# YuxinxinChen/dlrm-yx

Measured on AMD Instinct MI355X. Metric: DLRM samples/sec fwd+bwd at 1/2/4/8 MI355X; embedding HBM GB/s vs peak, higher is better.
Workload: dtype fp32; 1 GPU; mlperf_terabyte_synthetic; global_batch=2048, local_batch=2048, tables=26, rows_total=54063992, emb_dim=128, lookups_per_bag=1, optimizer=sgd, parallelism=table-sharded emb x1 + dp1, hip_graph=True, capture=whole, bot_sched=auto, tbe_role=True, bottom_parts=0, head_role=True, early_sort=True, feature_pad=False

## Files before the change

### dlrm-yx_amd/csrc/gemm.hip

```cpp
#include <cstdlib>
#include <cstring>
#include <type_traits>

#include "common.hpp"
#include "tbe_bwd_roles.hpp"

#ifndef DLRM_GEMM_STAMP
#define DLRM_GEMM_STAMP(slot)
#endif

namespace {

using f32x16 = __attribute__((ext_vector_type(16))) float;
using f32x4 = __attribute__((ext_vector_type(4))) float;
constexpr int kThreads = 256;
constexpr int kMaxSplit = 32;
constexpr int kMaxGroup = 6;
constexpr int64_t kTicketCap = 16384;
constexpr int kBK = 32;
constexpr int kRasterRows = 4;

struct GemmParams {
  int64_t M, N, K;
  float alpha;
// ... 6 lines not shown
  int epi;
  const float* bias;
  const float* aux;
  int64_t ldaux;
  int64_t ones_col;
  int layout;
  int tiles_m, tiles_n;
  int splits;
  int block0;
  int64_t kchunk;
  float* ws;
  int* counters;
  int mode;
  float* part;
  const float* alpha_dev;
};

struct GemmGroup {
  GemmParams p[kMaxGroup];
  int n;
  int total;
};

__device__ __forceinline__ int swz_kc(int r) {
  return ((r >> 1) & 7) ^ (((unsigned)((r & 15) - 4) < 8u) ? 2 : 0);
}

template <int MN, int BKT, bool KC, bool VEC, int NT, bool SWZ = false>
struct Stage {
  static_assert(!SWZ || (BKT % 32 == 0 && MN >= 32), "swizzled images: BKT 32 U, MN >= 32");
// ... 154 lines not shown
  asm("v_add_f32 %0, %1, %2" : "=v"(r) : "v"(a), "v"(b));
  return r;
}

__device__ __forceinline__ int xcd_remap(int bid, int nwg) {
  const int xcd = bid % 8;
  const int q = nwg / 8, r = nwg % 8;
  return (xcd < r ? xcd * (q + 1) : r * (q + 1) + (xcd - r) * q) + bid / 8;
}

__device__ __forceinline__ float apply_epilogue(const GemmParams& p, int64_t row, int64_t col,
                                                float v) {
  float* cp = p.C + row * p.ldc + col;
  switch (p.epi) {
    case DLRM_EPI_BIAS:
      v += p.bias[col];
      break;
    case DLRM_EPI_BIAS_RELU:
      v = fmaxf(v + p.bias[col], 0.f);
      break;
    case DLRM_EPI_RELU:
      v = fmaxf(v, 0.f);
      break;
    case DLRM_EPI_DRELU:
      v = p.aux[row * p.ldaux + col] > 0.f ? v : 0.f;
      break;
    case DLRM_EPI_SGD:
      v = *cp - v;
      break;
    case DLRM_EPI_ACCUM:
      v = *cp + v;
      break;
    default:
      break;
// ... 9 lines not shown
  else if constexpr (EPI == DLRM_EPI_RELU) return fmaxf(v, 0.f);
  else if constexpr (EPI == DLRM_EPI_DRELU) return aux > 0.f ? v : 0.f;
  else if constexpr (EPI == DLRM_EPI_SGD) return old - v;
  else if constexpr (EPI == DLRM_EPI_ACCUM) return old + v;
  else return v;
}

__device__ __forceinline__ float buf_ld(__amdgpu_buffer_rsrc_t r, int off) {
  return __builtin_bit_cast(float, __builtin_amdgcn_raw_buffer_load_b32(r, off, 0, 0));
}
__device__ __forceinline__ void buf_st(float v, __amdgpu_buffer_rsrc_t r, int off) {
  __builtin_amdgcn_raw_buffer_store_b32(__builtin_bit_cast(unsigned int, v), r, off, 0, 0);
}
constexpr int kOob = 0x7ffffff0;

template <int EPI, int NE>
__device__ __forceinline__ void store_elems(const GemmParams& p, const int (&row)[NE],
                                            const int (&col)[NE], const bool (&ok)[NE],
                                            const float (&v)[NE]) {
  const __amdgpu_buffer_rsrc_t rc = __builtin_amdgcn_make_buffer_rsrc(
      (void*)p.C, (short)0, (int)(((p.M - 1) * p.ldc + p.ldc) * 4), 0x00020000);
  int off[NE];
#pragma unroll
  for (int q = 0; q < NE; ++q)
    off[q] = ok[q] && row[q] < p.M ? (int)(((int64_t)row[q] * p.ldc + col[q]) * 4) : kOob;
  float old[NE], aux[NE], bias[NE];
#pragma unroll
  for (int q = 0; q < NE; ++q) old[q] = aux[q] = bias[q] = 0.f;
  if constexpr (EPI == DLRM_EPI_SGD || EPI == DLRM_EPI_ACCUM) {
#pragma unroll
    for (int q = 0; q < NE; ++q) old[q] = buf_ld(rc, off[q]);
  }
  if constexpr (EPI == DLRM_EPI_DRELU) {
    const __amdgpu_buffer_rsrc_t ra = __builtin_amdgcn_make_buffer_rsrc(
        (void*)p.aux, (short)0, (int)(((p.M - 1) * p.ldaux + p.ldaux) * 4), 0x00020000);
#pragma unroll
    for (int q = 0; q < NE; ++q)
      aux[q] = buf_ld(ra, ok[q] && row[q] < p.M ? (int)(((int64_t)row[q] * p.ldaux + col[q]) * 4)
                                                : kOob);
  }
  if constexpr (EPI == DLRM_EPI_BIAS || EPI == DLRM_EPI_BIAS_RELU) {
#pragma unroll
    for (int q = 0; q < NE; ++q) bias[q] = ok[q] ? p.bias[col[q]] : 0.f;
  }
#pragma unroll
  for (int q = 0; q < NE; ++q) buf_st(epi_value<EPI>(v[q], old[q], aux[q], bias[q]), rc, off[q]);
}

__device__ __forceinline__ bool epi_fits(const GemmParams& p) {
  const int64_t lim = 0x7ff00000LL;
  return (p.M + 256) * p.ldc * 4 < lim &&
         (p.epi != DLRM_EPI_DRELU || (p.M + 256) * p.ldaux * 4 < lim);
}

template <int NE>
__device__ __forceinline__ void store_elems_any(const GemmParams& p, const int (&row)[NE],
                                                const int (&col)[NE], const bool (&ok)[NE],
                                                const float (&v)[NE]) {
  switch (p.epi) {
    case DLRM_EPI_BIAS: return store_elems<DLRM_EPI_BIAS>(p, row, col, ok, v);
    case DLRM_EPI_BIAS_RELU: return store_elems<DLRM_EPI_BIAS_RELU>(p, row, col, ok, v);
    case DLRM_EPI_RELU: return store_elems<DLRM_EPI_RELU>(p, row, col, ok, v);
    case DLRM_EPI_DRELU: return store_elems<DLRM_EPI_DRELU>(p, row, col, ok, v);
    case DLRM_EPI_SGD: return store_elems<DLRM_EPI_SGD>(p, row, col, ok, v);
    case DLRM_EPI_ACCUM: return store_elems<DLRM_EPI_ACCUM>(p, row, col, ok, v);
    default: return store_elems<DLRM_EPI_STORE>(p, row, col, ok, v);
  }
}


template <int BM, int BN, int NV, int FM>
__device__ __forceinline__ bool splitk_reduce(const GemmParams& p, int tile, int split,
                                              float (&v)[NV], float (&rs)[FM], int rs_row0,
                                              int rs_stride, bool rs_owner, float* smem) {
  if (p.splits <= 1) return true;
  constexpr int REC = BM * BN + BM;
  static_assert(NV % 4 == 0, "record chunks are float4");
  using u32x4 = __attribute__((ext_vector_type(4))) unsigned int;
  const int tid = threadIdx.x;
  float* tile_base = p.ws + (int64_t)tile * p.splits * REC;
  const __amdgpu_buffer_rsrc_t rr = __builtin_amdgcn_make_buffer_rsrc(
      (void*)tile_base, (short)0, (int)(p.splits * REC * 4), 0x00020000);
// ... 52 lines not shown
    load_rec(s + 1, t1, r1);
    add_rec(t0, r0, s == 0);
    add_rec(t1, r1, false);
  }
  if (s < p.splits) {
    float4 t0[NV / 4];
    float r0[FM];
    load_rec(s, t0, r0);
    add_rec(t0, r0, s == 0);
  }
  return true;
}

template <int BM, int BN, int WGM, int WGN, bool RS, int FM, int FN>
__device__ __forceinline__ void finish_tile(const GemmParams& p, float alpha,
                                            const f32x4 (&acc)[FM][FN], float (&rs)[FM], int tile,
                                            int split, int tn, int64_t m0, int64_t n0,
                                            float* smem) {
  constexpr int WM = BM / WGM, WN = BN / WGN;
  const int tid = threadIdx.x;
  const int wave = tid >> 6;
  const int lane = tid & 63;
  const int kq = lane >> 4;
  const int l16 = lane & 15;
  const int wm0 = (wave / WGN) * WM;
  const int wn0 = (wave % WGN) * WN;
  const bool rs_owner = RS && tn == 0 && (wave % WGN) == 0 && kq == 0;

  constexpr int NV = FM * FN * 4;
  float v[NV];
#pragma unroll
  for (int i = 0; i < FM; ++i)
#pragma unroll
// ... 42 lines not shown
      float* rslab = p.part + (int64_t)p.splits * p.M * p.N + (int64_t)split * p.M;
#pragma unroll
      for (int i = 0; i < FM; ++i) {
        const int64_t row = m0 + wm0 + i * 16 + l16;
        if (row < p.M) rslab[row] = rs[i];
      }
    }
    return;
  }
  if (!splitk_reduce<BM, BN, NV, FM>(p, tile, split, v, rs, wm0 + l16, 16, rs_owner, smem))
    return;
  if (epi_fits(p)) {
    int row[NV], col[NV];
    bool ok[NV];
    float w[NV];
#pragma unroll
    for (int i = 0; i < FM; ++i)
#pragma unroll
      for (int j = 0; j < FN; ++j)
#pragma unroll
        for (int r = 0; r < 4; ++r) {
          const int q = (i * FN + j) * 4 + r;
          row[q] = (int)(m0 + wm0 + i * 16 + 4 * kq + r);
          col[q] = (int)(n0 + wn0 + j * 16 + l16);
          ok[q] = col[q] < p.N;
          w[q] = __fmul_rn(alpha, v[q]);
        }
    store_elems_any<NV>(p, row, col, ok, w);
    if constexpr (RS) {
      int rrow[FM], rcol[FM];
      bool rok[FM];
      float rw[FM];
#pragma unroll
      for (int i = 0; i < FM; ++i) {
        rrow[i] = (int)(m0 + wm0 + i * 16 + l16);
        rcol[i] = (int)p.ones_col;
        rok[i] = rs_owner;
        rw[i] = __fmul_rn(alpha, rs[i]);
      }
      store_elems_any<FM>(p, rrow, rcol, rok, rw);
    }
    return;
  }
#pragma unroll
  for (int i = 0; i < FM; ++i)
#pragma unroll
    for (int j = 0; j < FN; ++j) {
      const int64_t col = n0 + wn0 + j * 16 + l16;
#pragma unroll
      for (int r = 0; r < 4; ++r) {
        const int64_t row = m0 + wm0 + i * 16 + 4 * kq + r;
        if (row < p.M && col < p.N) apply_epilogue(p, row, col, alpha * v[(i * FN + j) * 4 + r]);
      }
    }
  if (rs_owner) {
// ... 158 lines not shown
    if (!last) {
      mfma_step(ca, cb, KL - 1);
      const int g = u * KL + KL - 1;
      if (g < NS) {
        put_one(g, nbuf);
        fetch_any(g, kt + 2, fast);
      }
      __builtin_amdgcn_sched_barrier(0);
    } else {
      __syncthreads();
      read_frags(nbuf, 0, na, nb);
      __builtin_amdgcn_sched_barrier(0);
      mfma_step(ca, cb, KL - 1);
    }
  };
  float a1[FM][KL], b1[FN][KL];
  if constexpr (U == 1) {
    const std::true_type fast{};
    const std::false_type slow{};
    for (int kt = 0; kt < nk; kt += 2) {
      if (kb32 + (kt + 3) * BKT <= kend32)
        subtile(kt, 0, a, b, a1, b1, fast);
      else
        subtile(kt, 0, a, b, a1, b1, slow);
      DLRM_GEMM_STAMP(2 + kt);
      if (kt + 1 >= nk) break;
      if (kb32 + (kt + 4) * BKT <= kend32)
        subtile(kt + 1, 0, a1, b1, a, b, fast);
      else
        subtile(kt + 1, 0, a1, b1, a, b, slow);
      DLRM_GEMM_STAMP(3 + kt);
    }
  } else {
    for (int kt = 0; kt < nk; ++kt) {
#pragma unroll
      for (int u = 0; u < U; u += 2) {
        subtile(kt, u, a, b, a1, b1, std::false_type{});
        subtile(kt, u + 1, a1, b1, a, b, std::false_type{});
      }
    }
  }

#pragma unroll
  for (int i = 0; i < FM; ++i) {
    rs[i] += __shfl_xor(rs[i], 16, 64);
    rs[i] += __shfl_xor(rs[i], 32, 64);
  }
  DLRM_GEMM_STAMP(-2);
  finish_tile<BM, BN, WGM, WGN, RS>(p, alpha, acc, rs, tile, split, tn, m0, n0, smem);
  DLRM_GEMM_STAMP(-1);
}

__device__ __forceinline__ void reduce_body(const GemmParams& p, int lb) {
  const float alpha = dlrm_resolve_lr(p.alpha_dev, p.alpha);
  const int64_t MN = p.M * p.N;
  const int64_t i = (int64_t)lb * blockDim.x + threadIdx.x;
  const int64_t n4 = MN / 4;
  const int S = p.splits;
  if (i < n4) {
    const float4* src = reinterpret_cast<const float4*>(p.part) + i;
    const int64_t stride = MN / 4;
    float4 acc = src[0];
    for (int s0 = 1; s0 < S; s0 += 8) {
      float4 t[8];
// ... 184 lines not shown
  int64_t M, N, K;
  float alpha;
  const float *A, *B;
  int64_t lda, ldb;
  float* C;
  int64_t ldc;
  int32_t epi;
  const float* bias;
  const float* aux;
  int64_t ldaux;
  int64_t ones_col;
  int32_t mode = DLRM_GEMM_FULL;
  int32_t splits = 0;
  float* part = nullptr;
  const float* alpha_dev = nullptr;
};

inline bool aligned16(const void* p) { return (reinterpret_cast<uintptr_t>(p) & 15) == 0; }

bool pipe_ok(const Desc& d) {
  const bool a_kc = !d.trans_a, b_kc = d.trans_b != 0;
  const int64_t a_ext = a_kc ? (d.M - 1) * d.lda + d.K : (d.K - 1) * d.lda + d.M;
  const int64_t b_ext = b_kc ? (d.N - 1) * d.ldb + d.K : (d.K - 1) * d.ldb + d.N;
  return aligned16(d.A) && aligned16(d.B) && d.lda % 4 == 0 && d.ldb % 4 == 0 && d.K % 4 == 0 &&
         (a_kc || d.M % 4 == 0) && (b_kc || d.N % 4 == 0) && a_ext * 4 < 0x7ff00000LL &&
         b_ext * 4 < 0x7ff00000LL;
}

int layout_of(const Desc& d) {
  const bool a_kc = !d.trans_a, b_kc = d.trans_b != 0;
// ... 24 lines not shown
  }
};

void plan_one(const Desc& d, Tile& t, Plan& pl) {
  t = Tile{64, 64, 2, 2};
  if (d.mode == DLRM_GEMM_REDUCE) {
    pl.splits = d.splits;
    pl.kchunk = 0;
    return;
  }
  if (d.mode == DLRM_GEMM_PARTIAL && d.splits > 0) {
    Desc q = d;
    q.mode = DLRM_GEMM_FULL;
    plan_one(q, t, pl);
    pl = make_plan(d.splits, d.K);
    return;
  }
  if (const int64_t tile = dlrm::tuning(DLRM_TUNE_GEMM_TILE)) {
    const int a = (int)(tile / 1000), b = (int)(tile % 1000);
    if (tile_ok(a, b, 2, 2)) t = Tile{a, b, 2, 2};
    const int64_t fs = dlrm::tuning(DLRM_TUNE_GEMM_SPLIT);
    pl = make_plan(fs > 0 ? fs : 1, d.K);
    return;
  }
  const bool use_table = true;
  if (use_table)
    for (const PlanEntry& e : kPlans)
      if (e.M == d.M && e.N == d.N && e.K == d.K && e.layout == layout_of(d)) {
        t = Tile{e.bm, e.bn, e.wm, e.wn};
        pl = make_plan(e.split, d.K);
// ... 53 lines not shown
  GemmGroup g{};
  g.n = n;
  WsCarver c(ws);
  int* tickets = c.take<int>(kTicketCap);
  int64_t tick = 0, blocks = 0;
  for (int i = 0; i < n; ++i) {
    GemmParams& p = g.p[i];
    p.M = d[i].M, p.N = d[i].N, p.K = d[i].K, p.alpha = d[i].alpha;
    p.A = d[i].A, p.lda = d[i].lda, p.B = d[i].B, p.ldb = d[i].ldb;
    p.C = d[i].C, p.ldc = d[i].ldc, p.epi = d[i].epi, p.bias = d[i].bias;
    p.aux = d[i].aux, p.ldaux = d[i].ldaux, p.ones_col = d[i].ones_col;
    p.layout = layout_of(d[i]);
    p.mode = d[i].mode;
    p.part = d[i].part;
    p.alpha_dev = d[i].alpha_dev;
    p.tiles_m = (int)dlrm::ceil_div(p.M, BM);
    p.tiles_n = (int)dlrm::ceil_div(p.N, BN);
    p.splits = pl[i].splits;
    p.kchunk = pl[i].kchunk > 0 ? pl[i].kchunk : kBK;
    p.block0 = (int)blocks;
    if (p.mode == DLRM_GEMM_REDUCE) {
      blocks += dlrm::ceil_div(p.M * p.N / 4 + (p.ones_col >= 0 ? p.M : 0), NT);
      continue;
    }
    if (p.splits > 1 && p.mode == DLRM_GEMM_FULL) {
      const int64_t tiles = (int64_t)p.tiles_m * p.tiles_n;
      p.counters = tickets + tick;
      p.ws = c.take<float>((size_t)tiles * p.splits * (BM * BN + BM));
      tick += tiles;
    }
// ... 37 lines not shown
#undef K_
    default:
      hipLaunchKernelGGL((gemm_group_kernel<BM, BN, WGM, WGN, 31, U>), grid, block, 0, st, g);
  }
  DLRM_LAUNCH_CHECK("dlrm_gemm_f32");
  return DLRM_OK;
}

int launch_generic(const Desc& d, hipStream_t st) {
  GemmParams p{};
  p.M = d.M, p.N = d.N, p.K = d.K, p.alpha = d.alpha;
  p.A = d.A, p.lda = d.lda, p.B = d.B, p.ldb = d.ldb;
  p.C = d.C, p.ldc = d.ldc, p.epi = d.epi, p.bias = d.bias;
  p.aux = d.aux, p.ldaux = d.ldaux, p.ones_col = d.ones_col;
  p.alpha_dev = d.alpha_dev;
  p.tiles_m = (int)dlrm::ceil_div(p.M, 64);
  p.tiles_n = (int)dlrm::ceil_div(p.N, 64);
  p.splits = 1;
  const bool a_kc = !d.trans_a, b_kc = d.trans_b != 0;
  const dim3 grid(p.tiles_m * p.tiles_n), block(kThreads);
  if (a_kc && b_kc)
    hipLaunchKernelGGL((gemm_generic_kernel<true, true>), grid, block, 0, st, p);
  else if (a_kc)
    hipLaunchKernelGGL((gemm_generic_kernel<true, false>), grid, block, 0, st, p);
  else if (b_kc)
    hipLaunchKernelGGL((gemm_generic_kernel<false, true>), grid, block, 0, st, p);
  else
    hipLaunchKernelGGL((gemm_generic_kernel<false, false>), grid, block, 0, st, p);
  DLRM_LAUNCH_CHECK("dlrm_gemm_f32 (generic)");
  if (d.ones_col >= 0) {
// ... 97 lines not shown
    return launch_group<32, 32>(m, q, pl, ws, ws_bytes, role, phase, st);
  if (t.bm == 32) return launch_group<32, 64>(m, q, pl, ws, ws_bytes, role, phase, st);
  if (t.bn == 32) return launch_group<64, 32>(m, q, pl, ws, ws_bytes, role, phase, st);
  return launch_group<64, 64>(m, q, pl, ws, ws_bytes, role, phase, st);
}

Desc desc_of(const dlrm_gemm_problem& g) {
  Desc d;
  d.trans_a = g.trans_a, d.trans_b = g.trans_b;
  d.M = g.M, d.N = g.N, d.K = g.K, d.alpha = g.alpha;
  d.A = g.A, d.lda = g.lda, d.B = g.B, d.ldb = g.ldb;
  d.C = g.C, d.ldc = g.ldc, d.epi = g.epilogue, d.bias = g.bias;
  d.aux = g.aux, d.ldaux = g.ld_aux, d.ones_col = g.ones_col;
  d.mode = g.mode, d.splits = g.splits, d.part = g.partial;
  d.alpha_dev = g.alpha_dev;
  return d;
}

}

extern "C" size_t dlrm_gemm_f32_workspace_size(int32_t trans_a, int32_t trans_b, int64_t M,
                                               int64_t N, int64_t K) {
  if (M <= 0 || N <= 0 || K <= 0) return 0;
  Desc d{};
  d.trans_a = trans_a, d.trans_b = trans_b, d.M = M, d.N = N, d.K = K;
  d.lda = ((trans_a ? M : K) + 3) / 4 * 4, d.ldb = ((trans_b ? K : N) + 3) / 4 * 4;
  d.A = d.B = reinterpret_cast<const float*>(256);
  d.ones_col = -1;
  return ws_for(1, &d);
}
// ... 67 lines not shown
```

### dlrm-yx_amd/csrc/mlp_rows.hpp

```cpp
#pragma once
#include "common.hpp"
#include "dlrm_hip.h"

namespace {

constexpr int kMlpRows = 16;
constexpr int kMlpWaves = 16;
constexpr int kMlpTiles = 2;
static_assert(kMlpTiles == 2, "mlp_rows_body dispatches mlp_kloop<1..2>");
constexpr int kMlpMaxK = 528;
constexpr int kMlpPitch = kMlpMaxK + 4;
constexpr int kMlpLdsFloats = 2 * kMlpRows * kMlpPitch + 4;

using mlp_f32x4 = __attribute__((ext_vector_type(4))) float;

struct MlpChain {
  int layers;
  int64_t rows;
  const float* X;
  int64_t ldx;
  int kin[DLRM_MLP_MAX_LAYERS];
  int nout[DLRM_MLP_MAX_LAYERS];
  const float* W[DLRM_MLP_MAX_LAYERS];
  int64_t ldw[DLRM_MLP_MAX_LAYERS];
  float* Y[DLRM_MLP_MAX_LAYERS];
  int64_t ldy[DLRM_MLP_MAX_LAYERS];
  int parts;
  int split;
  int* tickets;
};

constexpr int kMlpRing = 8;

template <int NTW>
__device__ __forceinline__ void mlp_kloop(mlp_f32x4 (&acc)[kMlpTiles], const float* in,
                                          __amdgpu_buffer_rsrc_t rw, int tb, int wave, int n,
                                          int kp, int64_t ldw, int nch, int l16, int kq) {
// ... 70 lines not shown
  const int64_t r0 = rblk * RB;
  float* in = lds;
  float* nx = lds + RB * P;
  {
    const int kp = mc.kin[0], kr4 = ((kp + 15) & ~15) / 4;
    for (int e = tid; e < RB * kr4; e += NT) {
      const int r = e / kr4, c4 = e - r * kr4;
      float4 v = make_float4(0.f, 0.f, 0.f, 0.f);
      if (r0 + r < mc.rows && 4 * c4 < kp)
        v = *reinterpret_cast<const float4*>(mc.X + (r0 + r) * mc.ldx + 4 * c4);
      *reinterpret_cast<float4*>(in + r * P + 4 * c4) = v;
    }
  }
  __syncthreads();
  for (int l = 0; l < mc.layers; ++l) {
    const int kp = mc.kin[l], n = mc.nout[l];
    const int nch = (kp + 15) / 16, ntile = (n + 15) / 16;
    const float* W = mc.W[l];
    const int64_t ldw = mc.ldw[l];
    const __amdgpu_buffer_rsrc_t rw = __builtin_amdgcn_make_buffer_rsrc(
        (void*)W, (short)0, (int)(((int64_t)(n - 1) * ldw + kp) * 4), 0x00020000);
    const bool split = parts > 1 && l == mc.split;
    const bool publish = split && l + 1 < mc.layers;
    const int tb = split ? q * ntile / parts : 0, te = split ? (q + 1) * ntile / parts : ntile;
    const int mt = te - tb;
    mlp_f32x4 acc[MT];
#pragma unroll
    for (int j = 0; j < MT; ++j) acc[j] = mlp_f32x4{0.f, 0.f, 0.f, 0.f};
    const int nt_w = mt > wave ? (mt - wave + NW - 1) / NW : 0;
    switch (nt_w) {
      case 1: mlp_kloop<1>(acc, in, rw, tb, wave, n, kp, ldw, nch, l16, kq); break;
      case 2: mlp_kloop<2>(acc, in, rw, tb, wave, n, kp, ldw, nch, l16, kq); break;
      default: break;
    }
    float* Y = mc.Y[l];
    const int64_t ldy = mc.ldy[l];
    const bool write_y = q == 0 || l >= mc.split;
    const int64_t nrow = mc.rows - r0 < RB ? mc.rows - r0 : RB;
    const __amdgpu_buffer_rsrc_t ry = __builtin_amdgcn_make_buffer_rsrc(
        (void*)(Y + r0 * ldy), (short)0, (int)(publish ? nrow * ldy * 4 : 0), 0x00020000);
#pragma unroll
    for (int j = 0; j < MT; ++j) {
      const int col = (tb + wave + j * NW) * 16 + l16;
      if (wave + j * NW < mt && col < n) {
#pragma unroll
        for (int r = 0; r < 4; ++r) {
          const int row = 4 * kq + r;
          const float v = fmaxf(acc[j][r], 0.f);
          nx[row * P + col] = v;
          if (publish) {
            if (row < nrow)
              __builtin_amdgcn_raw_buffer_store_b32(__builtin_bit_cast(unsigned int, v), ry,
                                                    (int)((row * ldy + col) * 4), 0, 16);
          } else if (write_y && r0 + row < mc.rows) {
            Y[(r0 + row) * ldy + col] = v;
          }
        }
      }
    }
    if (publish) {
      asm volatile("s_waitcnt vmcnt(0)" ::: "memory");
      __syncthreads();
      int* flag = reinterpret_cast<int*>(lds + 2 * RB * P);
// ... 37 lines not shown
  if (!c->X || !a16(c->X) || c->ldx % 4 != 0) return 0;
  mc.layers = c->layers;
  mc.rows = c->rows;
  mc.X = c->X;
  mc.ldx = c->ldx;
  for (int l = 0; l < c->layers; ++l) {
    const int64_t kin = c->in_width[l], n = c->out_width[l];
    if (kin < 1 || kin % 4 != 0 || ((kin + 15) & ~15) > kMlpMaxK) return 0;
    if (n < 1 || n > kMlpWaves * kMlpTiles * 16) return 0;
    if (l == 0 ? c->ldx < kin : kin != ((c->out_width[l - 1] + 1 + 3) / 4) * 4) return 0;
    if (!c->W[l] || !a16(c->W[l]) || c->ldw[l] % 4 != 0 || c->ldw[l] < kin) return 0;
    if (((n - 1) * c->ldw[l] + kin) * 4 >= 0x7ff00000LL) return 0;
    if (!c->Y[l] || c->ldy[l] < n) return 0;
    mc.kin[l] = (int)kin;
    mc.nout[l] = (int)n;
    mc.W[l] = c->W[l];
    mc.ldw[l] = c->ldw[l];
    mc.Y[l] = c->Y[l];
    mc.ldy[l] = c->ldy[l];
  }
  mc.parts = c->parts > 1 ? c->parts : 1;
  mc.split = c->split_layer;
  mc.tickets = c->tickets;
  if (mc.parts > 1) {
    if (mc.parts != 2 && mc.parts != 4) return 0;
    if (mc.split < 0 || mc.split >= c->layers) return 0;
    if ((c->out_width[mc.split] + 15) / 16 < mc.parts) return 0;
    if (mc.split + 1 < c->layers) {
      if (!c->tickets) return 0;
      if ((int64_t)kMlpRows * c->ldy[mc.split] * 4 >= 0x7ff00000LL) return 0;
// ... 11 lines not shown
```

### dlrm-yx_amd/dlrm_hip/_lib.py

```python
from __future__ import annotations

import ctypes
import os
from ctypes import c_float, c_int32, c_int64, c_size_t, c_uint64, c_void_p

_HERE = os.path.dirname(os.path.abspath(__file__))
ABI_VERSION = 14
LIB_PATH = os.environ.get("DLRM_HIP_LIB", os.path.join(_HERE, "libdlrm_hip.so"))


class DLRMHipUnavailable(RuntimeError):
    pass


class DLRMHipError(RuntimeError):

    def __init__(self, fn: str, code: int, msg: str):
        super().__init__(f"{fn} failed (status {code}): {msg}")
        self.code = code


class GemmProblem(ctypes.Structure):
    _fields_ = [("trans_a", c_int32), ("trans_b", c_int32), ("M", c_int64), ("N", c_int64),
                ("K", c_int64), ("alpha", c_float), ("A", c_void_p), ("lda", c_int64),
                ("B", c_void_p), ("ldb", c_int64), ("C", c_void_p), ("ldc", c_int64),
                ("epilogue", c_int32), ("bias", c_void_p), ("aux", c_void_p),
                ("ld_aux", c_int64), ("ones_col", c_int64), ("mode", c_int32),
                ("splits", c_int32), ("partial", c_void_p), ("alpha_dev", c_void_p)]


MLP_MAX_LAYERS = 4


class MlpChain(ctypes.Structure):
    _fields_ = [("layers", c_int32), ("rows", c_int64), ("X", c_void_p), ("ldx", c_int64),
                ("in_width", c_int64 * MLP_MAX_LAYERS), ("out_width", c_int64 * MLP_MAX_LAYERS),
                ("W", c_void_p * MLP_MAX_LAYERS), ("ldw", c_int64 * MLP_MAX_LAYERS),
                ("Y", c_void_p * MLP_MAX_LAYERS), ("ldy", c_int64 * MLP_MAX_LAYERS),
                ("parts", c_int32), ("split_layer", c_int32), ("tickets", c_void_p)]


class LaunchRole(ctypes.Structure):
    _fields_ = [("opaque", ctypes.c_uint64 * 32)]


class EvalStateC(ctypes.Structure):
    _fields_ = [("keys", c_void_p), ("capacity", c_int64), ("cursor", c_void_p),
                ("counts", c_void_p), ("error", c_void_p)]


P = c_void_p
SIGNATURES = {
    "dlrm_abi_version": (c_int32, []),
    "dlrm_last_error": (ctypes.c_char_p, []),
# ... 169 lines not shown
```

### dlrm-yx_amd/dlrm_hip/ops.py

```python
from __future__ import annotations

import ctypes
from typing import Optional, Sequence

import torch

from . import _lib

EPI_STORE, EPI_BIAS, EPI_BIAS_RELU, EPI_DRELU, EPI_SGD, EPI_ACCUM, EPI_RELU = range(7)
TBE_ERR_INDEX, TBE_ERR_TABLE_CAP = 1, 2


class TBEIndexError(IndexError):
    """Raised by check_tbe_errors: the reference's EmbeddingBag raises IndexError for an
    index outside its table; the device kernels skip such lookups and flag them."""


def check_tbe_errors(flag: torch.Tensor, reset: bool = True) -> None:
    v = int(flag.item())
    if reset:
        flag.zero_()
    if v & TBE_ERR_INDEX:
        raise TBEIndexError("embedding index out of range for its table (lookup skipped)")
    if v & TBE_ERR_TABLE_CAP:
# ... 143 lines not shown

def mlp_chain(X: torch.Tensor, layers, parts: int = 1, split_layer: int = -1,
              tickets: Optional[torch.Tensor] = None) -> "_lib.MlpChain":
    c = _lib.MlpChain()
    if parts > 1:
        if split_layer < 0:
            split_layer = max(range(len(layers)), key=lambda i: layers[i][2] * layers[i][0].shape[0])
        if tickets is None:
            tickets = torch.zeros((X.shape[0] + 15) // 16, dtype=torch.int32, device=X.device)
        c.parts, c.split_layer, c.tickets = int(parts), int(split_layer), tickets.data_ptr()
        c._keep = tickets
    c.layers = len(layers)
    c.rows = X.shape[0]
    c.X = X.data_ptr()
    c.ldx = X.stride(0)
    for i, (W, Y, kin) in enumerate(layers):
        c.in_width[i] = int(kin)
        c.out_width[i] = W.shape[0]
        c.W[i] = W.data_ptr()
        c.ldw[i] = W.stride(0)
        c.Y[i] = Y.data_ptr()
        c.ldy[i] = Y.stride(0)
    return c


def mlp_chain_supported(chain) -> bool:
    return bool(_lib.load().dlrm_mlp_chain_supported(ctypes.byref(chain)))


def mlp_chain_forward(chain, device=None) -> None:
    dev = device if device is not None else torch.cuda.current_device()
    _lib.call("dlrm_mlp_chain_forward", ctypes.cast(ctypes.byref(chain), ctypes.c_void_p),
# ... 386 lines not shown
    if A.stride(1) != 1 or B.stride(1) != 1:
        raise ValueError("gemm operands need unit inner stride")
    M = A.shape[1] if trans_a else A.shape[0]
    K = A.shape[0] if trans_a else A.shape[1]
    N = B.shape[0] if trans_b else B.shape[1]
    Kb = B.shape[1] if trans_b else B.shape[0]
    if K != Kb:
        raise ValueError(f"gemm inner dims differ: {K} vs {Kb}")
    if C is None:
        C = torch.empty((M, N if ones_col < 0 else max(N, ones_col + 1)), dtype=torch.float32,
                        device=A.device)
    if C.stride(1) != 1 or C.shape[0] != M or C.shape[1] < N:
        raise ValueError("gemm output must be [M, >= N] with unit inner stride")
    if ones_col >= 0 and not (N <= ones_col < C.shape[1]):
        raise ValueError("ones_col must be a column of C outside [0, N)")
    pr = _lib.GemmProblem(int(trans_a), int(trans_b), M, N, K,
                          0.0 if alpha_dev is not None else float(alpha), A.data_ptr(),
                          A.stride(0), B.data_ptr(), B.stride(0), C.data_ptr(), C.stride(0),
                          int(epilogue), bias.data_ptr() if bias is not None else None,
                          aux.data_ptr() if aux is not None else None,
                          aux.stride(0) if aux is not None else 0, int(ones_col),
                          GEMM_PARTIAL if partial is not None else GEMM_FULL, int(splits),
                          partial.data_ptr() if partial is not None else None, alpha_dev)
    return pr, C


def gemm_splits(pr, partial: bool = False, requested: int = 0) -> int:
    q = _lib.GemmProblem.from_buffer_copy(pr)
    if partial:
        q.mode = GEMM_PARTIAL
    q.splits = int(requested) if partial else 0
    return int(_lib.load().dlrm_gemm_f32_splits(ctypes.byref(q)))


def gemm_partial_bytes(M: int, N: int, splits: int) -> int:
    return _lib.query("dlrm_gemm_f32_partial_bytes", M, N, splits)


def sgd_job(param: torch.Tensor, grad: torch.Tensor, lr):
    _check_cuda(param, grad)
    lr_dev = _lr_dev(lr, "sgd_job: lr")
    n = param.numel()
    if grad.numel() != n or n % 4 or param.data_ptr() % 16 or grad.data_ptr() % 16:
        raise ValueError("sgd_job: flat fp32 tensors of equal size, numel % 4 == 0, 16-B aligned")
    return _lib.GemmProblem(0, 0, 1, n, 0, 0.0 if lr_dev is not None else float(lr), None, 0,
                            None, 0, param.data_ptr(), n, EPI_SGD, None, None, 0, -1,
                            GEMM_REDUCE, 1, grad.data_ptr(), lr_dev)


def reduce_problem(pr_partial):
    q = _lib.GemmProblem.from_buffer_copy(pr_partial)
    q.mode = GEMM_REDUCE
    return q


def _problems(prs):
    arr = (_lib.GemmProblem * len(prs))(*prs)
    return arr


def gemm_group_workspace_size(problems) -> int:
    return _lib.query("dlrm_gemm_f32_group_workspace_size", len(problems),
# ... 414 lines not shown
```

### dlrm-yx_amd/dlrm_hip/trainer.py

```python
from __future__ import annotations

import math
from dataclasses import dataclass, field
from typing import List, Optional, Sequence

import numpy as np
import torch
from torch.autograd.profiler import record_function

from . import ops
from .optim import check_lr_policy
from .sharders import shard


PRECISIONS = ("fp32", "bf16", "fp16")


def _pad4(n: int) -> int:
    return (int(n) + 3) // 4 * 4


def _precision(precision: str) -> str:
    if precision not in PRECISIONS:
        raise ValueError(f"precision {precision!r}: one of {PRECISIONS}")
# ... 1184 lines not shown
                graphs[key] = (fixed, self.capture_predict(fixed, metrics, precision=precision))
            fixed, run = graphs[key]
            fixed.X.copy_(batch.X)
            fixed.offsets.copy_(batch.offsets)
            fixed.indices.copy_(batch.indices)
            fixed.target.copy_(batch.target)
            run()
        self.check_errors()
        return metrics.compute(group=self.pg if self.world > 1 else None)

    def check_errors(self) -> None:
        ops.check_tbe_errors(self.tbe_error_flag)

    @staticmethod
    def _fwd(L: _Layer, h, out):
        return ops.gemm_problem(h[:, :L.Kp], L.W, trans_b=True, C=out, epilogue=ops.EPI_RELU)[0]

    @staticmethod
    def _dgrad(L: _Layer, g, inp, out):
        n = L.K if L.K % 4 == 0 else L.Kp
        if inp is not None:
            return ops.gemm_problem(g[:, :L.N], L.W[:, :n], C=out[:, :n], epilogue=ops.EPI_DRELU,
                                    aux=inp)[0]
        return ops.gemm_problem(g[:, :L.N], L.W[:, :n], C=out[:, :n])[0]

    @staticmethod
    def _wgrad(L: _Layer, g, inp, fused_opt, lr, **part):
        C = L.W if fused_opt else L.gW
        kw = dict(alpha=lr, epilogue=ops.EPI_SGD) if fused_opt else {}
        if L.K % 4 == 0:
            return ops.gemm_problem(g[:, :L.N], inp[:, :L.K], trans_a=True, C=C, ones_col=L.K,
# ... 10 lines not shown
        s = sp[key]
        if s <= 1:
            return self._wgrad(L, g, inp, fused_opt, lr), None
        parts = bufs.setdefault("partials", {})
        M, N = L.N, (L.K if L.K % 4 == 0 else L.Kp)
        need = ops.gemm_partial_bytes(M, N, s)
        if key not in parts or parts[key].numel() * 4 < need:
            parts[key] = torch.empty((need + 3) // 4, dtype=torch.float32, device=self.dev)
        pr = self._wgrad(L, g, inp, fused_opt, lr, partial=parts[key], splits=s)
        return pr, ops.reduce_problem(pr)

    def _bottom_chain(self, batch: Batch, bufs, sort_wgs: Optional[int] = None,
                      standalone: bool = False):
        if not self.fuse_bottom or (self.T_local == 0 and not standalone):
            return None
        layers = [(L.W, out, L.Kp) for L, out in zip(self.bot, bufs["bot_act"])]
        nrb = (batch.X.shape[0] + 15) // 16
        parts = self.bottom_parts
        others = self.T_local + 1 if sort_wgs is None else sort_wgs
        if parts <= 0:
            parts = next((p for p in (4, 2) if nrb * p + others <= self._cus), 1)
        widest = max(range(len(layers)), key=lambda i: layers[i][2] * layers[i][0].shape[0])
        if (layers[widest][0].shape[0] + 15) // 16 < parts:
            parts = 1
        if parts > 1:
            tk = bufs.get("mlp_tickets")
            if tk is None or tk.numel() < nrb:
                tk = bufs["mlp_tickets"] = torch.zeros(nrb, dtype=torch.int32,
                                                       device=self.dev)
            chain = ops.mlp_chain(batch.X, layers, parts=parts, split_layer=widest,
                                  tickets=tk)
# ... 109 lines not shown
```

### include/dlrm_hip.h

```cpp
#ifndef DLRM_HIP_H_
#define DLRM_HIP_H_

#include <stddef.h>
#include <stdint.h>

#ifdef __cplusplus
extern "C" {
#endif

typedef struct ihipStream_t* dlrm_stream_t;

enum dlrm_status {
  DLRM_OK = 0,
  DLRM_ERR_INVALID_ARG = 1,
  DLRM_ERR_SHAPE = 2,
  DLRM_ERR_UNSUPPORTED = 3,
  DLRM_ERR_WORKSPACE = 4,
  DLRM_ERR_HIP = 5
};

enum dlrm_epilogue {
  DLRM_EPI_STORE = 0,
  DLRM_EPI_BIAS = 1,
  DLRM_EPI_BIAS_RELU = 2,
  DLRM_EPI_DRELU = 3,
  DLRM_EPI_SGD = 4,
  DLRM_EPI_ACCUM = 5,
  DLRM_EPI_RELU = 6
};

enum dlrm_loss { DLRM_LOSS_MSE = 0, DLRM_LOSS_BCE = 1 };

enum dlrm_tbe_error {
  DLRM_TBE_ERR_INDEX = 1,
  DLRM_TBE_ERR_TABLE_CAP = 2
};

enum dlrm_qr_op { DLRM_QR_MULT = 0, DLRM_QR_ADD = 1, DLRM_QR_CONCAT = 2 };

#define DLRM_ABI_VERSION 14
int dlrm_abi_version(void);
const char* dlrm_last_error(void);

enum dlrm_tune_key {
  DLRM_TUNE_GEMM_TILE = 1,
  DLRM_TUNE_GEMM_SPLIT = 2,
  DLRM_TUNE_TBE_BLOCK = 3,
  DLRM_TUNE_TBE_SORT = 4,
  DLRM_TUNE_TBE_LEAN = 5,
  DLRM_TUNE_INTERACT_BWD = 6,
  DLRM_TUNE_INTERACT_FWD = 7,
  DLRM_TUNE_LINEAR16_TILE = 8,
  DLRM_TUNE_LINEAR16_DGRAD_TILE = 9,
  DLRM_TUNE_LINEAR16_WGRAD_TILE = 10,
  DLRM_TUNE_LINEAR16_WGRAD_SPLIT = 11
// ... 9 lines not shown
#define DLRM_MLP_MAX_LAYERS 4
typedef struct dlrm_mlp_chain {
  int32_t layers;
  int64_t rows;
  const float* X;
  int64_t ldx;
  int64_t in_width[DLRM_MLP_MAX_LAYERS];
  int64_t out_width[DLRM_MLP_MAX_LAYERS];
  const float* W[DLRM_MLP_MAX_LAYERS];
  int64_t ldw[DLRM_MLP_MAX_LAYERS];
  float* Y[DLRM_MLP_MAX_LAYERS];
  int64_t ldy[DLRM_MLP_MAX_LAYERS];
  int32_t parts;
  int32_t split_layer;
  int32_t* tickets;
} dlrm_mlp_chain;

int dlrm_mlp_chain_supported(const dlrm_mlp_chain* chain);

int dlrm_mlp_chain_forward(const dlrm_mlp_chain* chain, dlrm_stream_t stream);

int dlrm_tbe_forward_presort(const float* weights, int64_t D, const int64_t* row_base, int32_t T,
                             int32_t B, const void* indices, int32_t index_bits,
                             const void* offsets, int32_t offset_bits,
                             const float* per_sample_weights, float* out,
                             int64_t out_batch_stride, int64_t num_lookups, int64_t total_rows,
                             int64_t max_lookups_per_table, void* workspace,
                             size_t workspace_bytes, int32_t* error_flag,
                             const dlrm_mlp_chain* bottom, dlrm_stream_t stream);

// ... 157 lines not shown
  float alpha;
  const float* A;
  int64_t lda;
  const float* B;
  int64_t ldb;
  float* C;
  int64_t ldc;
  int32_t epilogue;
  const float* bias;
  const float* aux;
  int64_t ld_aux;
  int64_t ones_col;
  int32_t mode;
  int32_t splits;
  float* partial;
  const float* alpha_dev;
} dlrm_gemm_problem;

size_t dlrm_gemm_f32_group_workspace_size(int32_t n, const dlrm_gemm_problem* problems);
int32_t dlrm_gemm_f32_splits(const dlrm_gemm_problem* problem);
size_t dlrm_gemm_f32_partial_bytes(int64_t M, int64_t N, int32_t splits);
int dlrm_gemm_f32_group(int32_t n, const dlrm_gemm_problem* problems, void* workspace,
                        size_t workspace_bytes, dlrm_stream_t stream);
int dlrm_gemm_f32_group_role(int32_t n, const dlrm_gemm_problem* problems, void* workspace,
                             size_t workspace_bytes, const dlrm_launch_role* role,
                             int32_t phase, dlrm_stream_t stream);

size_t dlrm_colsum_workspace_size(int64_t M, int64_t N);
int dlrm_colsum_f32(int64_t M, int64_t N, const float* Y, int64_t ldy, const float* scale,
                    float alpha, float* out, int32_t accumulate, float* sgd_param, float lr,
// ... 171 lines not shown
```

Before: 5.418 million samples/s.

## Apply bias in GEMM epilogue instead of folded ones-column, prefetch epilogue operands

Forward MLP layers previously folded the bias into the weight matrix as an extra K column (Kp) multiplied against a ones column. They now run the GEMM over K only and add a strided bias (a weight column) in a BIAS_RELU epilogue, both in the grouped GEMM and in the fused bottom-MLP row kernel. Epilogue operands (bias, old C, aux) are factored into separate loads. Bias can be prefetched before the last K iteration to hide load latency, with an off-by-default prefetch path for the other operands. This drops the padded K work but adds strided bias loads and ABI changes.

```diff
diff --git a/dlrm-yx_amd/csrc/gemm.hip b/dlrm-yx_amd/csrc/gemm.hip
--- a/dlrm-yx_amd/csrc/gemm.hip
+++ b/dlrm-yx_amd/csrc/gemm.hip
@@ -44,6 +44,7 @@
   int mode;
   float* part;
   const float* alpha_dev;
+  int64_t ldbias;
 };
 
 struct GemmGroup {
@@ -228,10 +229,10 @@
   float* cp = p.C + row * p.ldc + col;
   switch (p.epi) {
     case DLRM_EPI_BIAS:
-      v += p.bias[col];
+      v += p.bias[col * p.ldbias];
       break;
     case DLRM_EPI_BIAS_RELU:
-      v = fmaxf(v + p.bias[col], 0.f);
+      v = fmaxf(v + p.bias[col * p.ldbias], 0.f);
       break;
     case DLRM_EPI_RELU:
       v = fmaxf(v, 0.f);
@@ -271,58 +272,107 @@
 }
 constexpr int kOob = 0x7ffffff0;
 
+template <int NE>
+__device__ __forceinline__ void load_operands(const GemmParams& p, const int (&row)[NE],
+                                              const int (&col)[NE], const bool (&ok)[NE],
+                                              float (&opnd)[NE]) {
+#pragma unroll
+  for (int q = 0; q < NE; ++q) opnd[q] = 0.f;
+  if (p.epi == DLRM_EPI_SGD || p.epi == DLRM_EPI_ACCUM || p.epi == DLRM_EPI_DRELU) {
+    const bool mask = p.epi == DLRM_EPI_DRELU;
+    const int64_t ld = mask ? p.ldaux : p.ldc;
+    const __amdgpu_buffer_rsrc_t rs = __builtin_amdgcn_make_buffer_rsrc(
+        (void*)(mask ? p.aux : p.C), (short)0, (int)(p.M * ld * 4), 0x00020000);
+#pragma unroll
+    for (int q = 0; q < NE; ++q)
+      opnd[q] = buf_ld(rs, ok[q] && row[q] < p.M ? (int)(((int64_t)row[q] * ld + col[q]) * 4)
+                                                 : kOob);
+  } else if (p.epi == DLRM_EPI_BIAS || p.epi == DLRM_EPI_BIAS_RELU) {
+    const __amdgpu_buffer_rsrc_t rs = __builtin_amdgcn_make_buffer_rsrc(
+        (void*)p.bias, (short)0, (int)(((p.N - 1) * p.ldbias + 1) * 4), 0x00020000);
+#pragma unroll
+    for (int q = 0; q < NE; ++q)
+      opnd[q] = buf_ld(rs, ok[q] ? (int)((int64_t)col[q] * p.ldbias * 4) : kOob);
+  }
+}
+
+template <int FN>
+__device__ __forceinline__ void load_bias(const GemmParams& p, int64_t n0w, int l16,
+                                          float (&bias)[FN]) {
+  const __amdgpu_buffer_rsrc_t rs = __builtin_amdgcn_make_buffer_rsrc(
+      (void*)p.bias, (short)0, (int)(((p.N - 1) * p.ldbias + 1) * 4), 0x00020000);
+#pragma unroll
+  for (int j = 0; j < FN; ++j) {
+    const int64_t col = n0w + j * 16 + l16;
+    bias[j] = buf_ld(rs, col < p.N ? (int)(col * p.ldbias * 4) : kOob);
+  }
+}
+
+__device__ __forceinline__ bool epi_has_bias(const GemmParams& p) {
+  return p.epi == DLRM_EPI_BIAS || p.epi == DLRM_EPI_BIAS_RELU;
+}
+
 template <int EPI, int NE>
 __device__ __forceinline__ void store_elems(const GemmParams& p, const int (&row)[NE],
                                             const int (&col)[NE], const bool (&ok)[NE],
-                                            const float (&v)[NE]) {
+                                            const float (&v)[NE], const float (&opnd)[NE]) {
   const __amdgpu_buffer_rsrc_t rc = __builtin_amdgcn_make_buffer_rsrc(
-      (void*)p.C, (short)0, (int)(((p.M - 1) * p.ldc + p.ldc) * 4), 0x00020000);
-  int off[NE];
-#pragma unroll
-  for (int q = 0; q < NE; ++q)
-    off[q] = ok[q] && row[q] < p.M ? (int)(((int64_t)row[q] * p.ldc + col[q]) * 4) : kOob;
-  float old[NE], aux[NE], bias[NE];
-#pragma unroll
-  for (int q = 0; q < NE; ++q) old[q] = aux[q] = bias[q] = 0.f;
-  if constexpr (EPI == DLRM_EPI_SGD || EPI == DLRM_EPI_ACCUM) {
-#pragma unroll
-    for (int q = 0; q < NE; ++q) old[q] = buf_ld(rc, off[q]);
-  }
-  if constexpr (EPI == DLRM_EPI_DRELU) {
-    const __amdgpu_buffer_rsrc_t ra = __builtin_amdgcn_make_buffer_rsrc(
-        (void*)p.aux, (short)0, (int)(((p.M - 1) * p.ldaux + p.ldaux) * 4), 0x00020000);
-#pragma unroll
-    for (int q = 0; q < NE; ++q)
-      aux[q] = buf_ld(ra, ok[q] && row[q] < p.M ? (int)(((int64_t)row[q] * p.ldaux + col[q]) * 4)
-                                                : kOob);
-  }
-  if constexpr (EPI == DLRM_EPI_BIAS || EPI == DLRM_EPI_BIAS_RELU) {
-#pragma unroll
-    for (int q = 0; q < NE; ++q) bias[q] = ok[q] ? p.bias[col[q]] : 0.f;
-  }
-#pragma unroll
-  for (int q = 0; q < NE; ++q) buf_st(epi_value<EPI>(v[q], old[q], aux[q], bias[q]), rc, off[q]);
+      (void*)p.C, (short)0, (int)(p.M * p.ldc * 4), 0x00020000);
+#pragma unroll
+  for (int q = 0; q < NE; ++q) {
+    const int off = ok[q] && row[q] < p.M ? (int)(((int64_t)row[q] * p.ldc + col[q]) * 4) : kOob;
+    buf_st(epi_value<EPI>(v[q], opnd[q], opnd[q], opnd[q]), rc, off);
+  }
 }
 
 __device__ __forceinline__ bool epi_fits(const GemmParams& p) {
   const int64_t lim = 0x7ff00000LL;
+  const bool bias = p.epi == DLRM_EPI_BIAS || p.epi == DLRM_EPI_BIAS_RELU;
   return (p.M + 256) * p.ldc * 4 < lim &&
-         (p.epi != DLRM_EPI_DRELU || (p.M + 256) * p.ldaux * 4 < lim);
+         (p.epi != DLRM_EPI_DRELU || (p.M + 256) * p.ldaux * 4 < lim) &&
+         (!bias || (p.N + 256) * p.ldbias * 4 < lim);
 }
 
 template <int NE>
 __device__ __forceinline__ void store_elems_any(const GemmParams& p, const int (&row)[NE],
                                                 const int (&col)[NE], const bool (&ok)[NE],
-                                                const float (&v)[NE]) {
+                                                const float (&v)[NE], const float (&opnd)[NE]) {
   switch (p.epi) {
-    case DLRM_EPI_BIAS: return store_elems<DLRM_EPI_BIAS>(p, row, col, ok, v);
-    case DLRM_EPI_BIAS_RELU: return store_elems<DLRM_EPI_BIAS_RELU>(p, row, col, ok, v);
-    case DLRM_EPI_RELU: return store_elems<DLRM_EPI_RELU>(p, row, col, ok, v);
-    case DLRM_EPI_DRELU: return store_elems<DLRM_EPI_DRELU>(p, row, col, ok, v);
-    case DLRM_EPI_SGD: return store_elems<DLRM_EPI_SGD>(p, row, col, ok, v);
-    case DLRM_EPI_ACCUM: return store_elems<DLRM_EPI_ACCUM>(p, row, col, ok, v);
-    default: return store_elems<DLRM_EPI_STORE>(p, row, col, ok, v);
-  }
+    case DLRM_EPI_BIAS: return store_elems<DLRM_EPI_BIAS>(p, row, col, ok, v, opnd);
+    case DLRM_EPI_BIAS_RELU: return store_elems<DLRM_EPI_BIAS_RELU>(p, row, col, ok, v, opnd);
+    case DLRM_EPI_RELU: return store_elems<DLRM_EPI_RELU>(p, row, col, ok, v, opnd);
+    case DLRM_EPI_DRELU: return store_elems<DLRM_EPI_DRELU>(p, row, col, ok, v, opnd);
+    case DLRM_EPI_SGD: return store_elems<DLRM_EPI_SGD>(p, row, col, ok, v, opnd);
+    case DLRM_EPI_ACCUM: return store_elems<DLRM_EPI_ACCUM>(p, row, col, ok, v, opnd);
+    default: return store_elems<DLRM_EPI_STORE>(p, row, col, ok, v, opnd);
+  }
+}
+
+template <int FM, int FN>
+__device__ __forceinline__ void tile_coords(const GemmParams& p, int64_t m0, int64_t n0, int wm0,
+                                            int wn0, int kq, int l16, int (&row)[FM * FN * 4],
+                                            int (&col)[FM * FN * 4], bool (&ok)[FM * FN * 4]) {
+#pragma unroll
+  for (int i = 0; i < FM; ++i)
+#pragma unroll
+    for (int j = 0; j < FN; ++j)
+#pragma unroll
+      for (int r = 0; r < 4; ++r) {
+        const int q = (i * FN + j) * 4 + r;
+        row[q] = (int)(m0 + wm0 + i * 16 + 4 * kq + r);
+        col[q] = (int)(n0 + wn0 + j * 16 + l16);
+        ok[q] = col[q] < p.N;
+      }
+}
+
+#ifndef DLRM_GEMM_PREFETCH_OPS
+#define DLRM_GEMM_PREFETCH_OPS 0
+#endif
+__device__ __forceinline__ bool epi_prefetch(const GemmParams& p) {
+  return p.splits <= 1 && p.mode == DLRM_GEMM_FULL && epi_fits(p);
+}
+__device__ __forceinline__ bool epi_prefetch_ops(const GemmParams& p) {
+  return DLRM_GEMM_PREFETCH_OPS != 0 && epi_prefetch(p) && !epi_has_bias(p);
 }
 
 
@@ -405,9 +455,10 @@
 
 template <int BM, int BN, int WGM, int WGN, bool RS, int FM, int FN>
 __device__ __forceinline__ void finish_tile(const GemmParams& p, float alpha,
-                                            const f32x4 (&acc)[FM][FN], float (&rs)[FM], int tile,
-                                            int split, int tn, int64_t m0, int64_t n0,
-                                            float* smem) {
+                                            const f32x4 (&acc)[FM][FN], float (&rs)[FM],
+                                            float (&opnd)[FM * FN * 4], float (&bias)[FN],
+                                            bool bias_ready, int tile, int split, int tn,
+                                            int64_t m0, int64_t n0, float* smem) {
   constexpr int WM = BM / WGM, WN = BN / WGN;
   const int tid = threadIdx.x;
   const int wave = tid >> 6;
@@ -480,19 +531,18 @@
     int row[NV], col[NV];
     bool ok[NV];
     float w[NV];
-#pragma unroll
-    for (int i = 0; i < FM; ++i)
-#pragma unroll
-      for (int j = 0; j < FN; ++j)
-#pragma unroll
-        for (int r = 0; r < 4; ++r) {
-          const int q = (i * FN + j) * 4 + r;
-          row[q] = (int)(m0 + wm0 + i * 16 + 4 * kq + r);
-          col[q] = (int)(n0 + wn0 + j * 16 + l16);
-          ok[q] = col[q] < p.N;
-          w[q] = __fmul_rn(alpha, v[q]);
-        }
-    store_elems_any<NV>(p, row, col, ok, w);
+    tile_coords<FM, FN>(p, m0, n0, wm0, wn0, kq, l16, row, col, ok);
+    if (epi_has_bias(p)) {
+      if (!bias_ready) load_bias<FN>(p, n0 + wn0, l16, bias);
+#pragma unroll
+      for (int q = 0; q < NV; ++q) opnd[q] = bias[(q / 4) % FN];
+    } else if (!epi_prefetch_ops(p)) {
+      load_operands<NV>(p, row, col, ok, opnd);
+    }
+#pragma unroll
+    for (int q = 0; q < NV; ++q)
+      w[q] = __fmul_rn(alpha, v[q]);
+    store_elems_any<NV>(p, row, col, ok, w, opnd);
     if constexpr (RS) {
       int rrow[FM], rcol[FM];
       bool rok[FM];
@@ -504,7 +554,9 @@
         rok[i] = rs_owner;
         rw[i] = __fmul_rn(alpha, rs[i]);
       }
-      store_elems_any<FM>(p, rrow, rcol, rok, rw);
+      float ro[FM];
+      load_operands<FM>(p, rrow, rcol, rok, ro);
+      store_elems_any<FM>(p, rrow, rcol, rok, rw, ro);
     }
     return;
   }
@@ -693,11 +745,33 @@
       mfma_step(ca, cb, KL - 1);
     }
   };
+  float opnd[FM * FN * 4];
+#pragma unroll
+  for (int q = 0; q < FM * FN * 4; ++q) opnd[q] = 0.f;
+  constexpr bool BIAS_PRE = A_KC && B_KC;
+  const bool bias_ready = BIAS_PRE && epi_prefetch(p) && epi_has_bias(p);
+  const bool prefetch = bias_ready || epi_prefetch_ops(p);
+  float bias[FN];
+#pragma unroll
+  for (int j = 0; j < FN; ++j) bias[j] = 0.f;
+  auto fetch_operands = [&]() {
+    int kqv = kq, lv = l16;
+    asm volatile("" : "+v"(kqv), "+v"(lv));
+    if (bias_ready) {
+      load_bias<FN>(p, n0 + wn0, lv, bias);
+    } else if (epi_prefetch_ops(p)) {
+      int row[FM * FN * 4], col[FM * FN * 4];
+      bool ok[FM * FN * 4];
+      tile_coords<FM, FN>(p, m0, n0, wm0, wn0, kqv, lv, row, col, ok);
+      load_operands<FM * FN * 4>(p, row, col, ok, opnd);
+    }
+  };
   float a1[FM][KL], b1[FN][KL];
   if constexpr (U == 1) {
     const std::true_type fast{};
     const std::false_type slow{};
     for (int kt = 0; kt < nk; kt += 2) {
+      if (prefetch && kt + 2 >= nk) fetch_operands();
       if (kb32 + (kt + 3) * BKT <= kend32)
         subtile(kt, 0, a, b, a1, b1, fast);
       else
@@ -712,6 +786,7 @@
     }
   } else {
     for (int kt = 0; kt < nk; ++kt) {
+      if (prefetch && kt + 1 >= nk) fetch_operands();
 #pragma unroll
       for (int u = 0; u < U; u += 2) {
         subtile(kt, u, a, b, a1, b1, std::false_type{});
@@ -726,7 +801,8 @@
     rs[i] += __shfl_xor(rs[i], 32, 64);
   }
   DLRM_GEMM_STAMP(-2);
-  finish_tile<BM, BN, WGM, WGN, RS>(p, alpha, acc, rs, tile, split, tn, m0, n0, smem);
+  finish_tile<BM, BN, WGM, WGN, RS>(p, alpha, acc, rs, opnd, bias, bias_ready, tile, split, tn,
+                                    m0, n0, smem);
   DLRM_GEMM_STAMP(-1);
 }
 
@@ -941,6 +1017,7 @@
   int32_t splits = 0;
   float* part = nullptr;
   const float* alpha_dev = nullptr;
+  int64_t ldbias = 1;
 };
 
 inline bool aligned16(const void* p) { return (reinterpret_cast<uintptr_t>(p) & 15) == 0; }
@@ -995,6 +1072,14 @@
     q.mode = DLRM_GEMM_FULL;
     plan_one(q, t, pl);
     pl = make_plan(d.splits, d.K);
+    return;
+  }
+  if (d.ldbias > 1 && (d.epi == DLRM_EPI_BIAS || d.epi == DLRM_EPI_BIAS_RELU)) {
+    Desc q = d;
+    q.K += 4;
+    q.ldbias = 1;
+    plan_one(q, t, pl);
+    pl = make_plan(pl.splits, d.K);
     return;
   }
   if (const int64_t tile = dlrm::tuning(DLRM_TUNE_GEMM_TILE)) {
@@ -1078,6 +1163,7 @@
     p.mode = d[i].mode;
     p.part = d[i].part;
     p.alpha_dev = d[i].alpha_dev;
+    p.ldbias = d[i].ldbias;
     p.tiles_m = (int)dlrm::ceil_div(p.M, BM);
     p.tiles_n = (int)dlrm::ceil_div(p.N, BN);
     p.splits = pl[i].splits;
@@ -1145,6 +1231,7 @@
   p.C = d.C, p.ldc = d.ldc, p.epi = d.epi, p.bias = d.bias;
   p.aux = d.aux, p.ldaux = d.ldaux, p.ones_col = d.ones_col;
   p.alpha_dev = d.alpha_dev;
+  p.ldbias = d.ldbias;
   p.tiles_m = (int)dlrm::ceil_div(p.M, 64);
   p.tiles_n = (int)dlrm::ceil_div(p.N, 64);
   p.splits = 1;
@@ -1272,6 +1359,7 @@
   d.aux = g.aux, d.ldaux = g.ld_aux, d.ones_col = g.ones_col;
   d.mode = g.mode, d.splits = g.splits, d.part = g.partial;
   d.alpha_dev = g.alpha_dev;
+  d.ldbias = g.ld_bias > 0 ? g.ld_bias : 1;
   return d;
 }
 
diff --git a/dlrm-yx_amd/csrc/mlp_rows.hpp b/dlrm-yx_amd/csrc/mlp_rows.hpp
--- a/dlrm-yx_amd/csrc/mlp_rows.hpp
+++ b/dlrm-yx_amd/csrc/mlp_rows.hpp
@@ -21,6 +21,7 @@
   int64_t ldx;
   int kin[DLRM_MLP_MAX_LAYERS];
   int nout[DLRM_MLP_MAX_LAYERS];
+  int bcol[DLRM_MLP_MAX_LAYERS];
   const float* W[DLRM_MLP_MAX_LAYERS];
   int64_t ldw[DLRM_MLP_MAX_LAYERS];
   float* Y[DLRM_MLP_MAX_LAYERS];
@@ -121,7 +122,8 @@
   }
   __syncthreads();
   for (int l = 0; l < mc.layers; ++l) {
-    const int kp = mc.kin[l], n = mc.nout[l];
+    const int bc = mc.bcol[l];
+    const int kp = bc > 0 ? bc : mc.kin[l], n = mc.nout[l];
     const int nch = (kp + 15) / 16, ntile = (n + 15) / 16;
     const float* W = mc.W[l];
     const int64_t ldw = mc.ldw[l];
@@ -135,6 +137,12 @@
 #pragma unroll
     for (int j = 0; j < MT; ++j) acc[j] = mlp_f32x4{0.f, 0.f, 0.f, 0.f};
     const int nt_w = mt > wave ? (mt - wave + NW - 1) / NW : 0;
+    float bias[MT];
+#pragma unroll
+    for (int j = 0; j < MT; ++j) {
+      const int col = (tb + wave + j * NW) * 16 + l16;
+      bias[j] = (bc > 0 && wave + j * NW < mt && col < n) ? W[col * ldw + bc] : 0.f;
+    }
     switch (nt_w) {
       case 1: mlp_kloop<1>(acc, in, rw, tb, wave, n, kp, ldw, nch, l16, kq); break;
       case 2: mlp_kloop<2>(acc, in, rw, tb, wave, n, kp, ldw, nch, l16, kq); break;
@@ -153,7 +161,7 @@
 #pragma unroll
         for (int r = 0; r < 4; ++r) {
           const int row = 4 * kq + r;
-          const float v = fmaxf(acc[j][r], 0.f);
+          const float v = fmaxf(bc > 0 ? acc[j][r] + bias[j] : acc[j][r], 0.f);
           nx[row * P + col] = v;
           if (publish) {
             if (row < nrow)
@@ -221,6 +229,9 @@
     if (!c->Y[l] || c->ldy[l] < n) return 0;
     mc.kin[l] = (int)kin;
     mc.nout[l] = (int)n;
+    const int64_t bc = c->bias_col[l];
+    if (bc != 0 && (bc < 4 || bc % 4 != 0 || bc >= kin)) return 0;
+    mc.bcol[l] = (int)bc;
     mc.W[l] = c->W[l];
     mc.ldw[l] = c->ldw[l];
     mc.Y[l] = c->Y[l];
diff --git a/dlrm-yx_amd/dlrm_hip/_lib.py b/dlrm-yx_amd/dlrm_hip/_lib.py
--- a/dlrm-yx_amd/dlrm_hip/_lib.py
+++ b/dlrm-yx_amd/dlrm_hip/_lib.py
@@ -5,7 +5,7 @@
 from ctypes import c_float, c_int32, c_int64, c_size_t, c_uint64, c_void_p
 
 _HERE = os.path.dirname(os.path.abspath(__file__))
-ABI_VERSION = 14
+ABI_VERSION = 15
 LIB_PATH = os.environ.get("DLRM_HIP_LIB", os.path.join(_HERE, "libdlrm_hip.so"))
 
 
@@ -26,7 +26,8 @@
                 ("B", c_void_p), ("ldb", c_int64), ("C", c_void_p), ("ldc", c_int64),
                 ("epilogue", c_int32), ("bias", c_void_p), ("aux", c_void_p),
                 ("ld_aux", c_int64), ("ones_col", c_int64), ("mode", c_int32),
-                ("splits", c_int32), ("partial", c_void_p), ("alpha_dev", c_void_p)]
+                ("splits", c_int32), ("partial", c_void_p), ("ld_bias", c_int64),
+                ("alpha_dev", c_void_p)]
 
 
 MLP_MAX_LAYERS = 4
@@ -37,7 +38,8 @@
                 ("in_width", c_int64 * MLP_MAX_LAYERS), ("out_width", c_int64 * MLP_MAX_LAYERS),
                 ("W", c_void_p * MLP_MAX_LAYERS), ("ldw", c_int64 * MLP_MAX_LAYERS),
                 ("Y", c_void_p * MLP_MAX_LAYERS), ("ldy", c_int64 * MLP_MAX_LAYERS),
-                ("parts", c_int32), ("split_layer", c_int32), ("tickets", c_void_p)]
+                ("parts", c_int32), ("split_layer", c_int32), ("tickets", c_void_p),
+                ("bias_col", c_int64 * MLP_MAX_LAYERS)]
 
 
 class LaunchRole(ctypes.Structure):
diff --git a/dlrm-yx_amd/dlrm_hip/ops.py b/dlrm-yx_amd/dlrm_hip/ops.py
--- a/dlrm-yx_amd/dlrm_hip/ops.py
+++ b/dlrm-yx_amd/dlrm_hip/ops.py
@@ -181,8 +181,9 @@
     c.rows = X.shape[0]
     c.X = X.data_ptr()
     c.ldx = X.stride(0)
-    for i, (W, Y, kin) in enumerate(layers):
+    for i, (W, Y, kin, *bcol) in enumerate(layers):
         c.in_width[i] = int(kin)
+        c.bias_col[i] = int(bcol[0]) if bcol else 0
         c.out_width[i] = W.shape[0]
         c.W[i] = W.data_ptr()
         c.ldw[i] = W.stride(0)
@@ -599,6 +600,9 @@
         raise ValueError("gemm output must be [M, >= N] with unit inner stride")
     if ones_col >= 0 and not (N <= ones_col < C.shape[1]):
         raise ValueError("ones_col must be a column of C outside [0, N)")
+    if bias is not None and (bias.dim() != 1 or bias.shape[0] < N or
+                             (N > 1 and bias.stride(0) < 1)):
+        raise ValueError("gemm bias must be 1-D with >= N elements and a positive stride")
     pr = _lib.GemmProblem(int(trans_a), int(trans_b), M, N, K,
                           0.0 if alpha_dev is not None else float(alpha), A.data_ptr(),
                           A.stride(0), B.data_ptr(), B.stride(0), C.data_ptr(), C.stride(0),
@@ -606,7 +610,8 @@
                           aux.data_ptr() if aux is not None else None,
                           aux.stride(0) if aux is not None else 0, int(ones_col),
                           GEMM_PARTIAL if partial is not None else GEMM_FULL, int(splits),
-                          partial.data_ptr() if partial is not None else None, alpha_dev)
+                          partial.data_ptr() if partial is not None else None,
+                          max(int(bias.stride(0)), 1) if bias is not None else 0, alpha_dev)
     return pr, C
 
 
@@ -630,7 +635,7 @@
         raise ValueError("sgd_job: flat fp32 tensors of equal size, numel % 4 == 0, 16-B aligned")
     return _lib.GemmProblem(0, 0, 1, n, 0, 0.0 if lr_dev is not None else float(lr), None, 0,
                             None, 0, param.data_ptr(), n, EPI_SGD, None, None, 0, -1,
-                            GEMM_REDUCE, 1, grad.data_ptr(), lr_dev)
+                            GEMM_REDUCE, 1, grad.data_ptr(), 0, lr_dev)
 
 
 def reduce_problem(pr_partial):
diff --git a/dlrm-yx_amd/dlrm_hip/trainer.py b/dlrm-yx_amd/dlrm_hip/trainer.py
--- a/dlrm-yx_amd/dlrm_hip/trainer.py
+++ b/dlrm-yx_amd/dlrm_hip/trainer.py
@@ -1222,7 +1222,12 @@
 
     @staticmethod
     def _fwd(L: _Layer, h, out):
-        return ops.gemm_problem(h[:, :L.Kp], L.W, trans_b=True, C=out, epilogue=ops.EPI_RELU)[0]
+        folded = ops.gemm_problem(h[:, :L.Kp], L.W, trans_b=True, C=out,
+                                  epilogue=ops.EPI_RELU)[0]
+        if L.K % 32 == 0 and ops.gemm_splits(folded) <= 1:
+            return ops.gemm_problem(h[:, :L.K], L.W[:, :L.K], trans_b=True, C=out,
+                                    epilogue=ops.EPI_BIAS_RELU, bias=L.b)[0]
+        return folded
 
     @staticmethod
     def _dgrad(L: _Layer, g, inp, out):
@@ -1263,7 +1268,8 @@
                       standalone: bool = False):
         if not self.fuse_bottom or (self.T_local == 0 and not standalone):
             return None
-        layers = [(L.W, out, L.Kp) for L, out in zip(self.bot, bufs["bot_act"])]
+        layers = [(L.W, out, L.Kp) + ((L.K,) if L.K % 16 == 0 else ())
+                  for L, out in zip(self.bot, bufs["bot_act"])]
         nrb = (batch.X.shape[0] + 15) // 16
         parts = self.bottom_parts
         others = self.T_local + 1 if sort_wgs is None else sort_wgs
diff --git a/include/dlrm_hip.h b/include/dlrm_hip.h
--- a/include/dlrm_hip.h
+++ b/include/dlrm_hip.h
@@ -38,7 +38,7 @@
 
 enum dlrm_qr_op { DLRM_QR_MULT = 0, DLRM_QR_ADD = 1, DLRM_QR_CONCAT = 2 };
 
-#define DLRM_ABI_VERSION 14
+#define DLRM_ABI_VERSION 15
 int dlrm_abi_version(void);
 const char* dlrm_last_error(void);
 
@@ -78,6 +78,7 @@
   int32_t parts;
   int32_t split_layer;
   int32_t* tickets;
+  int64_t bias_col[DLRM_MLP_MAX_LAYERS];
 } dlrm_mlp_chain;
 
 int dlrm_mlp_chain_supported(const dlrm_mlp_chain* chain);
@@ -265,6 +266,7 @@
   int32_t mode;
   int32_t splits;
   float* partial;
+  int64_t ld_bias;
   const float* alpha_dev;
 } dlrm_gemm_problem;
 
```

Result: no change. 5.403 million samples/s (-0.3%).
